# RustAudio/lewton

Hardware: AMD Instinct MI355X
Metric: audio packets/sec (44.1 kHz stereo, 2048-pt long blocks) (higher is better)
Workload: dtype f32; 1 GPU; BASELINE configs[1]: batches of 4096 synthetic 44.1 kHz stereo long-block (n=2048) packets per GPU = 256 streams x 16 consecutive packets, 8 batches rotated, records resident in HBM; streams_per_batch=256, channels=2, blocksize=2048, output=i16 planar, kernels=k_long, parity=unchecked (bench.py --full checks the timed batch against the oracle), parallelism=streams sharded across GPUs, no collectives

## Files before the change

### lewton_amd/csrc/lw_kernels_long.hip

```cpp
#include <algorithm>
#include <cstddef>
#include <mutex>

#include "lw_fast.hpp"
#include "lw_kernels.hpp"
#include "lw_pcm_store.inc"

#define LW_WG (64 * LW_FAST_WAVES)
#define LW_PRIO_FLOOR 2
#define LW_PRIO_IMDCT 0
#define LW_PRIO_FINISH 3
#define LW_FLOOR_FIRST_FROM 7
#define LW_IMDCT_PRIO_LATE 12
#define LW_PRIO_PACE 0
#define LW_PRIO_READY 3
#define LW_SCR_BYTES 4096u
#define LW_PUB_BYTES 4096u
#define LW_LDS_BYTES (LWI_TOTAL + LW_FAST_WAVES * (LW_SCR_BYTES + LW_PUB_BYTES) + 3 * LW_FAST_WAVES * 4)

#include "lw_stamps.inc"

struct LwFastArgs {
	const float *residue;
	const uint16_t *floors;
// ... 11 lines not shown
	float *td;
	float *halo;
	float *edge;
	void *out;
	uint32_t state_stride, state_chan_stride;
	uint32_t edge_n;
	const float *tabA;
	const uint16_t *sid12;
	uint32_t pre[LW_FAST_WAVES];
};
static_assert(offsetof(LwFastArgs, waves) == 48, "kernel reads waves[] through the kernarg segment pointer");

typedef unsigned int uint2_t __attribute__((ext_vector_type(2)));

__device__ __forceinline__ void lds_fence()
{
	asm volatile("" ::: "memory");
}

typedef __attribute__((address_space(3))) const float *lds_cfloat_ptr;
__device__ __forceinline__ float lds_abs_f32(uint32_t byte_addr)
{
	return *reinterpret_cast<lds_cfloat_ptr>((uintptr_t)byte_addr);
}

__device__ __forceinline__ float2_t lds2(const char *base, uint32_t byte_off)
{
	return *reinterpret_cast<const float2_t *>(base + byte_off);
}

__device__ __forceinline__ float4_t lds4(const char *base, uint32_t byte_off)
{
	return *reinterpret_cast<const float4_t *>(base + byte_off);
}

#define LW_PK(name, op, mods)                                                              \
	__device__ __forceinline__ float2_t name(float2_t a, float2_t b)                       \
	{                                                                                      \
		float2_t d;                                                                        \
		asm(op " %0, %1, %2 " mods : "=v"(d) : "v"(a), "v"(b));                            \
		return d;                                                                          \
	}
LW_PK(pk_add, "v_pk_add_f32", "")
LW_PK(pk_sub, "v_pk_add_f32", "neg_lo:[0,1] neg_hi:[0,1]")
LW_PK(pk_add_A2, "v_pk_add_f32", "op_sel:[0,1] op_sel_hi:[1,0] neg_lo:[0,1]")
LW_PK(pk_add_A3, "v_pk_add_f32", "op_sel:[1,1] op_sel_hi:[0,0] neg_lo:[0,1] neg_hi:[1,0]")
LW_PK(pk_add_A4, "v_pk_add_f32", "op_sel:[0,0] op_sel_hi:[1,1] neg_lo:[1,0] neg_hi:[0,1]")
LW_PK(pk_add_A5, "v_pk_add_f32", "op_sel:[1,0] op_sel_hi:[1,0] neg_lo:[0,1]")
LW_PK(pk_add_A6, "v_pk_add_f32", "op_sel:[0,1] op_sel_hi:[1,0] neg_hi:[0,1]")
LW_PK(pk_add_A7, "v_pk_add_f32", "neg_hi:[0,1]")
LW_PK(pk_add_A8, "v_pk_add_f32", "neg_lo:[0,1]")
LW_PK(pk_add_A9, "v_pk_add_f32", "neg_lo:[0,1] neg_hi:[1,0]")
LW_PK(pk_mul, "v_pk_mul_f32", "")
LW_PK(pk_mul_M1, "v_pk_mul_f32", "op_sel:[0,0] op_sel_hi:[1,0]")
LW_PK(pk_mul_M2, "v_pk_mul_f32", "op_sel:[1,1] op_sel_hi:[0,1] neg_hi:[0,1]")
LW_PK(pk_mul_M3, "v_pk_mul_f32", "op_sel:[0,1] op_sel_hi:[0,0]")
LW_PK(pk_mul_M4, "v_pk_mul_f32", "op_sel:[0,0] op_sel_hi:[0,1] neg_hi:[0,1]")
LW_PK(pk_mul_M5, "v_pk_mul_f32", "op_sel:[1,1] op_sel_hi:[1,0] neg_lo:[1,0] neg_hi:[1,0]")
LW_PK(pk_mul_M6, "v_pk_mul_f32", "op_sel:[1,0] op_sel_hi:[1,1] neg_lo:[1,0]")
LW_PK(pk_mul_M7, "v_pk_mul_f32", "op_sel:[0,1] op_sel_hi:[1,1]")
LW_PK(pk_mul_M8, "v_pk_mul_f32", "op_sel:[1,0] op_sel_hi:[0,0] neg_lo:[0,1]")
LW_PK(pk_mul_M9, "v_pk_mul_f32", "op_sel:[1,1] op_sel_hi:[1,0] neg_hi:[1,0]")
LW_PK(pk_mul_M10, "v_pk_mul_f32", "op_sel:[0,0] op_sel_hi:[0,1] neg_lo:[0,1] neg_hi:[0,1]")
LW_PK(pk_mul_M12lo, "v_pk_mul_f32", "op_sel:[0,1] op_sel_hi:[0,0]")
LW_PK(pk_mul_M12hi, "v_pk_mul_f32", "op_sel:[1,1] op_sel_hi:[1,0]")

// ... 195 lines not shown
	    : "+v"(m0), "+v"(a0), "+v"(m1), "+v"(a1), "+v"(m2), "+v"(a2), "+v"(m3), "+v"(a3), "=&v"(t0), "=&v"(t1), "=&v"(t2), "=&v"(t3),
	      "=&s"(c0), "=&s"(c1), "=&s"(c2), "=&s"(c3), "=&s"(d0), "=&s"(d1), "=&s"(d2), "=&s"(d3));
}

struct ItemRegs {
	uint32_t res_off, floor_off, out_off, src_arg;
	int32_t state_out;
	uint32_t halo_out, src_kind, flags;
	uint32_t pkt;
};

struct Pref {
	float4_t r[2][4];
	uint32_t fe[2];
};


__device__ __forceinline__ void issue_floor_loads(const LwFastArgs &F, const ItemRegs &it, const LwFastUnit &un, uint32_t lane,
		Pref &p)
{
	const uint16_t *f0 = F.floors + it.floor_off + (uint32_t)un.ch_a * F.fstride;
	p.fe[0] = lane < un.F_a ? (uint32_t)f0[lane] : 0u;
	p.fe[1] = 0u;
	if (un.ch_b >= 0) {
		const uint16_t *f1 = F.floors + it.floor_off + (uint32_t)un.ch_b * F.fstride;
		p.fe[1] = lane < un.F_b ? (uint32_t)f1[lane] : 0u;
	}
}

template <bool PAIR = false, bool NT = true>
__device__ __forceinline__ void issue_residue_loads(const LwFastArgs &F, const ItemRegs &it, const LwFastUnit &un,
		uint32_t lane, Pref &p)
{
	const float4_t *s0 = reinterpret_cast<const float4_t *>(F.residue + it.res_off + (uint32_t)un.ch_a * 1024u);
#pragma unroll
	for (int x = 0; x < 4; x++)
		p.r[0][x] = NT ? __builtin_nontemporal_load(&s0[64 * x + lane]) : s0[64 * x + lane];
	if (PAIR || un.ch_b >= 0) {
		const float4_t *s1 = reinterpret_cast<const float4_t *>(F.residue + it.res_off + (uint32_t)un.ch_b * 1024u);
#pragma unroll
		for (int x = 0; x < 4; x++)
			p.r[1][x] = NT ? __builtin_nontemporal_load(&s1[64 * x + lane]) : s1[64 * x + lane];
	}
}

template <bool NT = true>
__device__ __forceinline__ void issue_loads(const LwFastArgs &F, const ItemRegs &it, const LwFastUnit &un, uint32_t lane, Pref &p)
{
	issue_residue_loads<false, NT>(F, it, un, lane, p);
	issue_floor_loads(F, it, un, lane, p);
}

struct PreRegs {
	float4_t t[2][4];
};

__device__ __forceinline__ void issue_pre_loads(const LwFastArgs &F, const ItemRegs &it, uint32_t prog, uint32_t lane, PreRegs &q)
{
#pragma unroll
	for (int k = 0; k < 2; k++) {
		const uint32_t c = (prog >> (8 * k)) & 0xffu;
		if (c != LW_PRE_NO_CH) {
			const float4_t *s = reinterpret_cast<const float4_t *>(F.residue + it.res_off + c * 1024u);
#pragma unroll
			for (int x = 0; x < 4; x++)
				q.t[k][x] = s[64 * x + lane];
		} else {
#pragma unroll
			for (int x = 0; x < 4; x++)
				asm volatile("" : "=v"(q.t[k][x]));
		}
	}
}

#define LW_FLOOR_W0 2097153.0f
// ... 79 lines not shown
		ent[(b) & 1][3] = lds4(t, sw.y >> 16);                                         \
	} while (0)
#define LW_SP_XI(b)                                                                    \
	do {                                                                               \
		_Pragma("unroll") for (int j = 0; j < 4; j++) {                                \
			fl[(b) & 1][j] = floor_bin(kf0 + (float)(256 * ((b) & 3) + j), ent[(b) & 1][j]); \
		}                                                                              \
	} while (0)
#define LW_SP_M(b)                                                                     \
	do {                                                                               \
		float4_t &rr = r[(b) >> 2][(b) & 3];                                           \
		const float2_t lo2 = pk_mul(float2_t{fl[(b) & 1][0], fl[(b) & 1][1]}, float2_t{rr.x, rr.y}); \
		const float2_t hi2 = pk_mul(float2_t{fl[(b) & 1][2], fl[(b) & 1][3]}, float2_t{rr.z, rr.w}); \
		rr = float4_t{lo2.x, lo2.y, hi2.x, hi2.y};                                     \
	} while (0)
	LW_SP_G(0);
	LW_SP_G(1);
	__builtin_amdgcn_sched_barrier(0);
#pragma unroll
	for (int b = 0; b < 8; b++) {
		LW_SP_XI(b);
		if (b + 2 < 8)
			LW_SP_G(b + 2);
		if (b >= 1)
			LW_SP_M(b - 1);
		__builtin_amdgcn_sched_barrier(0);
	}
	LW_SP_M(7);
#undef LW_SP_G
#undef LW_SP_XI
#undef LW_SP_M
}

__device__ __forceinline__ void floor_values(const char *img, const char *sc, uint32_t lane, uint32_t fslot, bool unused,
		float4_t (&fl)[4])
{
	if (unused) {
#pragma unroll
		for (int x = 0; x < 4; x++)
			fl[x] = float4_t{0.0f, 0.0f, 0.0f, 0.0f};
		return;
	}
	const float kf0 = (float)(4 * (int)lane);
#pragma unroll
	for (int x = 0; x < 4; x++) {
		const uint2_t sw = *reinterpret_cast<const uint2_t *>(img + LWI_SID16 + 8u * ((fslot * 4 + x) * 64u + lane));
		const uint32_t s16[4] = {sw.x & 0xffffu, sw.x >> 16, sw.y & 0xffffu, sw.y >> 16};
#pragma unroll
		for (int j = 0; j < 4; j++) {
			fl[x][j] = floor_bin(kf0 + (float)(256 * x + j), lds4(sc, s16[j]));
		}
	}
}

template <int NCH>
__device__ __forceinline__ void floor_phase(const LwFastArgs &F, const char *img, char *sc, uint32_t lane, const LwFastUnit &un,
		const uint32_t (&fe)[2], float4_t (&fl)[2][4])
{
	__builtin_amdgcn_s_setprio(LW_PRIO_FLOOR);
	const bool unused0 = floor_table(F, img, sc, lane, fe[0], un.floor_a, un.F_a);
	bool unused1 = false;
	if (NCH == 2)
		unused1 = floor_table(F, img, sc + 1024, lane, fe[1], un.floor_b, un.F_b);
	lds_fence();
	floor_values(img, sc, lane, un.floor_a, unused0, fl[0]);
	if (NCH == 2)
		floor_values(img, sc + 1024, lane, un.floor_b, unused1, fl[1]);
	lds_fence();
	__builtin_amdgcn_s_setprio(0);
}

template <int NCH>
__device__ __forceinline__ void stage_b(const LwFastArgs &F, const char *img, uint32_t lane, const float4_t (&r)[2][4],
		float2_t (&P)[2][8])
{
	const uint32_t mirror = (63u - lane) << 2;
	float2_t au[4], al[4];
#pragma unroll
	for (int x = 0; x < 4; x++) {
		const uint32_t m = 64u * x + lane;
		au[x] = lds2(img + LWI_APAIR, 8u * m);
		al[x] = lds2(img + LWI_APAIR, 8u * (511u - m));
	}
#pragma unroll
	for (int c = 0; c < NCH; c++) {
		float2_t U[4];
		step1x2(r[c][0], au[0], al[0], r[c][1], au[1], al[1], U[0], P[c][0], U[1], P[c][1]);
		step1x2(r[c][2], au[2], al[2], r[c][3], au[3], al[3], U[2], P[c][2], U[3], P[c][3]);
#pragma unroll
		for (int x = 0; x < 4; x++) {
			P[c][7 - x].x = __int_as_float(__builtin_amdgcn_ds_bpermute(mirror, __float_as_int(U[x].x)));
			P[c][7 - x].y = __int_as_float(__builtin_amdgcn_ds_bpermute(mirror, __float_as_int(U[x].y)));
		}
	}
	float2_t s2[4], l0[2], l1;
#pragma unroll
	for (int x = 0; x < 4; x++)
		s2[x] = lds2(img + LWI_TW_S2, 8u * (64u * x + lane));
	l0[0] = lds2(img + LWI_TW_L0, 8u * lane);
	l0[1] = lds2(img + LWI_TW_L0, 8u * (64u + lane));
// ... 239 lines not shown
	float2_t P0[8], P1[8];
	TwC tc;
	{
		TwB tb;
		load_tw_b(img, lane, tb);
		stage_b1(tb, lane, r[0], P0);
		stage_b1(tb, lane, r[1], P1);
		load_tw_c(img, lane, tc);
		t2_inreg(P0);
		t2_inreg(P1);
		__builtin_amdgcn_sched_barrier(0);
	}
	stage_c1(tc, P0);
	__builtin_amdgcn_sched_barrier(0);
	const float a2s = *reinterpret_cast<const float *>(img + LWI_A2);
	const float2_t a2 = float2_t{a2s, a2s};
	t3_inreg(P0);
	stage_c1(tc, P1);
	__builtin_amdgcn_sched_barrier(0);
	t3_inreg(P1);
	stage_d_block(a2, P0);
	__builtin_amdgcn_sched_barrier(0);
	t4_write(sc, lane, P0);
	__builtin_amdgcn_sched_barrier(0);
	stage_e1(img, sc, lane, R[0]);
	stage_d_block(a2, P1);
	__builtin_amdgcn_sched_barrier(0);
	t4_write(sc, lane, P1);
	__builtin_amdgcn_sched_barrier(0);
	stage_e1(img, sc, lane, R[1]);
	__builtin_amdgcn_sched_barrier(0);
}

__device__ __forceinline__ void decouple_pair(Pref &pf)
{
#pragma unroll
	for (int x = 0; x < 4; x++) {
		float m[4] = {pf.r[0][x].x, pf.r[0][x].y, pf.r[0][x].z, pf.r[0][x].w};
		float a[4] = {pf.r[1][x].x, pf.r[1][x].y, pf.r[1][x].z, pf.r[1][x].w};
		decouple4(m[0], a[0], m[1], a[1], m[2], a[2], m[3], a[3]);
		pf.r[0][x] = float4_t{m[0], m[1], m[2], m[3]};
		pf.r[1][x] = float4_t{a[0], a[1], a[2], a[3]};
	}
}

__device__ __forceinline__ void couple_quad(float4_t &M, float4_t &A)
{
	float m[4] = {M.x, M.y, M.z, M.w};
	float a[4] = {A.x, A.y, A.z, A.w};
	decouple4_branchy(m[0], a[0], m[1], a[1], m[2], a[2], m[3], a[3]);
	M = float4_t{m[0], m[1], m[2], m[3]};
	A = float4_t{a[0], a[1], a[2], a[3]};
}

__device__ __forceinline__ void apply_pre(uint32_t prog, Pref &pf, PreRegs &q)
{
	const uint32_t n = prog >> 28;
#pragma unroll
	for (int x = 0; x < 4; x++) {
		float4_t v0 = pf.r[0][x], v1 = pf.r[1][x], v2 = q.t[0][x], v3 = q.t[1][x];
#pragma nounroll
		for (uint32_t i = 0; i < n; i++) {
			switch ((prog >> (16u + 4u * i)) & 0xfu) {
			case 0x1: couple_quad(v0, v1); break;
			case 0x2: couple_quad(v0, v2); break;
			case 0x3: couple_quad(v0, v3); break;
			case 0x4: couple_quad(v1, v0); break;
			case 0x6: couple_quad(v1, v2); break;
			case 0x7: couple_quad(v1, v3); break;
			case 0x8: couple_quad(v2, v0); break;
			case 0x9: couple_quad(v2, v1); break;
			case 0xb: couple_quad(v2, v3); break;
			case 0xc: couple_quad(v3, v0); break;
			case 0xd: couple_quad(v3, v1); break;
			case 0xe: couple_quad(v3, v2); break;
			default: break;
			}
		}
		pf.r[0][x] = v0;
		pf.r[1][x] = v1;
	}
}

template <int NCH, bool SPLIT = false>
__device__ __forceinline__ void spectrum_fused(const LwFastArgs &F, const char *img, char *sc, uint32_t lane,
		const LwFastUnit &un, Pref &pf)
{
	__builtin_amdgcn_s_setprio(LW_PRIO_FLOOR);
	const bool unused0 = floor_table(F, img, sc, lane, pf.fe[0], un.floor_a, un.F_a);
	bool unused1 = false;
	if (NCH == 2)
		unused1 = floor_table(F, img, sc + 1024, lane, pf.fe[1], un.floor_b, un.F_b);
	lds_fence();
	if (NCH == 2 && un.coupled)
		decouple_pair(pf);
	if (SPLIT && NCH == 1 && un.coupled >= LW_UNIT_SPLIT_MAG) {
		if (un.coupled == LW_UNIT_SPLIT_ANG) {
#pragma unroll
			for (int x = 0; x < 4; x++) {
				const float4_t t = pf.r[0][x];
				pf.r[0][x] = pf.r[1][x];
				pf.r[1][x] = t;
			}
			decouple_pair(pf);
#pragma unroll
			for (int x = 0; x < 4; x++)
				pf.r[0][x] = pf.r[1][x];
		} else {
			decouple_pair(pf);
		}
	}
	if (NCH == 2 && !unused0 && !unused1) {
		spectrum_pair(img, sc, lane, un.floor_a, un.floor_b, pf.r);
	} else {
		spectrum(F, img, sc, lane, un.floor_a, unused0, pf.r[0]);
		if (NCH == 2)
			spectrum(F, img, sc + 1024, lane, un.floor_b, unused1, pf.r[1]);
	}
	lds_fence();
}

__device__ __forceinline__ void spectrum_ready(const LwFastUnit &un, Pref &pf, const float4_t (&fl)[2][4])
{
	if (un.coupled)
		decouple_pair(pf);
#pragma unroll
	for (int c = 0; c < 2; c++)
#pragma unroll
		for (int x = 0; x < 4; x++) {
			const float2_t lo2 = pk_mul(float2_t{fl[c][x].x, fl[c][x].y}, float2_t{pf.r[c][x].x, pf.r[c][x].y});
			const float2_t hi2 = pk_mul(float2_t{fl[c][x].z, fl[c][x].w}, float2_t{pf.r[c][x].z, pf.r[c][x].w});
			pf.r[c][x] = float4_t{lo2.x, lo2.y, hi2.x, hi2.y};
		}
}

template <int NCH, int UP = 0>
__device__ __forceinline__ void long_imdct(const LwFastArgs &F, const char *img, char *sc, uint32_t lane, Pref &pf,
		float2_t (&R)[2][2][4])
{
	if (__builtin_amdgcn_readfirstlane(threadIdx.x >> 6) >= LW_IMDCT_PRIO_LATE)
		__builtin_amdgcn_s_setprio(LW_PRIO_IMDCT + 1 + UP);
	else
		__builtin_amdgcn_s_setprio(LW_PRIO_IMDCT + UP);
	if (NCH == 2) {
		imdct_pair(img, sc, lane, pf.r, R);
		return;
	}
	float2_t P[2][8];
	stage_b<NCH>(F, img, lane, pf.r, P);
#pragma unroll
	for (int c = 0; c < NCH; c++)
		t2_inreg(P[c]);
	stage_c<NCH>(F, img, lane, P);
#pragma unroll
	for (int c = 0; c < NCH; c++) {
		t3_inreg(P[c]);
	}
	{
		const float a2s = *reinterpret_cast<const float *>(img + LWI_A2);
		const float2_t a2 = float2_t{a2s, a2s};
#pragma unroll
		for (int c = 0; c < NCH; c++)
			stage_d_block(a2, P[c]);
	}
#pragma unroll
	for (int c = 0; c < NCH; c++) {
		t4_write(sc, lane, P[c]);
		lds_fence();
#pragma unroll
		for (int c2 = 0; c2 < 2; c2++) {
			TwidE te;
			te.Cq = lds4(img + LWI_C4, 16u * (64u * c2 + lane));
			te.Bl = lds4(img + LWI_B_LO, 16u * (64u * c2 + lane));
// ... 6 lines not shown

template <int NCH>
__device__ __forceinline__ void publish(char *dst, uint32_t lane, const float2_t (&R)[2][2][4])
{
#pragma unroll
	for (int c = 0; c < 2; c++)
		if (c < NCH) {
#pragma unroll
			for (int c2 = 0; c2 < 2; c2++)
				*reinterpret_cast<float4_t *>(dst + 2048 * c + 16u * (64u * c2 + lane)) =
					float4_t{R[c][c2][0].y, R[c][c2][1].y, R[c][c2][2].y, R[c][c2][3].y};
		}
}

#define LW_PB_LO0(c) float4_t{R[c][0][3].y, R[c][0][2].y, R[c][1][3].y, R[c][1][2].y}
#define LW_PB_LO1(c) float4_t{R[c][1][1].y, R[c][1][0].y, R[c][0][1].y, R[c][0][0].y}

struct PrevHalf {
	float2_t pp[2][2];
};

__device__ __forceinline__ void prev_from_lds(const char *src, uint32_t lane, PrevHalf &h)
{
#pragma unroll
	for (int c2 = 0; c2 < 2; c2++) {
		const float4_t v = *reinterpret_cast<const float4_t *>(src + 16u * (64u * c2 + lane));
		h.pp[c2][0] = float2_t{v.x, v.y};
		h.pp[c2][1] = float2_t{v.z, v.w};
	}
}

__device__ __forceinline__ void prev_from_global(const float *g, uint32_t lane, PrevHalf &h)
{
	const float4_t g0 = *reinterpret_cast<const float4_t *>(g + 4u * lane);
	const float4_t g1 = *reinterpret_cast<const float4_t *>(g + 508u - 4u * lane);
	h.pp[0][1] = float2_t{g0.y, g0.x};
	h.pp[1][1] = float2_t{g0.w, g0.z};
	h.pp[1][0] = float2_t{g1.y, g1.x};
	h.pp[0][0] = float2_t{g1.w, g1.z};
}

__device__ __forceinline__ void ola_pack_i16(const char *img, uint32_t lane, const float2_t (&Rc)[2][4], const PrevHalf &h,
		uint32_t (&D)[4][2])
{
	float2_t O[2][4];
#pragma unroll
	for (int c2 = 0; c2 < 2; c2++) {
		const float4_t w0 = lds4(img + LWI_WIN, 32u * (64u * c2 + lane));
		const float4_t w1 = lds4(img + LWI_WIN, 32u * (64u * c2 + lane) + 16u);
		ola_block<true>(Rc[c2], h.pp[c2][0], h.pp[c2][1], w0, w1, O[c2]);
	}
	typedef short short2_t __attribute__((ext_vector_type(2)));
	union {
		short2_t s;
		uint32_t u;
	} a;
#define LW_PKI(d, v0, v1) a.s = __builtin_amdgcn_cvt_pk_i16((int)(v0), (int)(v1)), d = a.u
	LW_PKI(D[0][0], O[0][3].x, O[0][2].x);
	LW_PKI(D[0][1], O[1][3].x, O[1][2].x);
	LW_PKI(D[1][0], O[1][1].x, O[1][0].x);
	LW_PKI(D[1][1], O[0][1].x, O[0][0].x);
	LW_PKI(D[2][0], O[0][0].y, O[0][1].y);
	LW_PKI(D[2][1], O[1][0].y, O[1][1].y);
	LW_PKI(D[3][0], O[1][2].y, O[1][3].y);
	LW_PKI(D[3][1], O[0][2].y, O[0][3].y);
#undef LW_PKI
}

__device__ __forceinline__ void store_interleaved2(const LwFastArgs &F, uint32_t lane, uint32_t out_off,
		const uint32_t (&L)[4][2], const uint32_t (&R)[4][2])
{
	int16_t *o = reinterpret_cast<int16_t *>(F.out) + out_off;
	const uint32_t pos[4] = {4u * lane, 508u - 4u * lane, 512u + 4u * lane, 1020u - 4u * lane};
#pragma unroll
	for (int g = 0; g < 4; g++) {
		const uint32_t d0 = __builtin_amdgcn_perm(R[g][0], L[g][0], 0x05040100u);
		const uint32_t d1 = __builtin_amdgcn_perm(R[g][0], L[g][0], 0x07060302u);
		const uint32_t d2 = __builtin_amdgcn_perm(R[g][1], L[g][1], 0x05040100u);
		const uint32_t d3 = __builtin_amdgcn_perm(R[g][1], L[g][1], 0x07060302u);
		store16_wt(o + 2u * pos[g], float4_t{__uint_as_float(d0), __uint_as_float(d1), __uint_as_float(d2), __uint_as_float(d3)});
	}
}

__device__ __forceinline__ void ola_quads_f32(const char *img, uint32_t lane, const float2_t (&Rc)[2][4], const PrevHalf &h, float4_t (&V)[4])
{
	float2_t O[2][4];
#pragma unroll
	for (int c2 = 0; c2 < 2; c2++) {
		const float4_t w0 = lds4(img + LWI_WIN, 32u * (64u * c2 + lane));
		const float4_t w1 = lds4(img + LWI_WIN, 32u * (64u * c2 + lane) + 16u);
		ola_block<false>(Rc[c2], h.pp[c2][0], h.pp[c2][1], w0, w1, O[c2]);
	}
	const LwQuads q = pcm_quads(O);
#pragma unroll
	for (int g = 0; g < 4; g++)
		V[g] = float4_t{q.v[g][0], q.v[g][1], q.v[g][2], q.v[g][3]};
}

__device__ __forceinline__ void store_interleaved2_f32(const LwFastArgs &F, uint32_t lane, uint32_t out_off, const float4_t (&L)[4],
		const float4_t (&R)[4])
{
	float *o = reinterpret_cast<float *>(F.out) + out_off;
	const bool odd = (lane & 1u) != 0;
#pragma unroll
	for (int g = 0; g < 4; g++) {
		const uint32_t b = 256u * (uint32_t)g;
#pragma unroll
		for (int h = 0; h < 2; h++) {
			const uint32_t k = 32u * (uint32_t)h + (lane >> 1);
			const int src = (int)((g & 1) ? 63u - k : k) << 2;
#define LW_BP(v) __int_as_float(__builtin_amdgcn_ds_bpermute(src, __float_as_int(v)))
			const float lx = LW_BP(L[g].x), ly = LW_BP(L[g].y), lz = LW_BP(L[g].z), lw = LW_BP(L[g].w);
			const float rx = LW_BP(R[g].x), ry = LW_BP(R[g].y), rz = LW_BP(R[g].z), rw = LW_BP(R[g].w);
#undef LW_BP
			const float4_t v = odd ? float4_t{lz, rz, lw, rw} : float4_t{lx, rx, ly, ry};
			store16_wt(o + 2u * (b + 128u * (uint32_t)h + 2u * lane), v);
		}
	}
}

template <int FMT>
__device__ __forceinline__ void ola_store(const LwFastArgs &F, const char *img, uint32_t lane, int chn,
		uint32_t out_off, const float2_t (&Rc)[2][4], const PrevHalf &h, uint32_t mch = 1024u)
{
	float2_t O[2][4];
#pragma unroll
	for (int c2 = 0; c2 < 2; c2++) {
		const float4_t w0 = lds4(img + LWI_WIN, 32u * (64u * c2 + lane));
		const float4_t w1 = lds4(img + LWI_WIN, 32u * (64u * c2 + lane) + 16u);
		ola_block<!lw_out_f32(FMT)>(Rc[c2], h.pp[c2][0], h.pp[c2][1], w0, w1, O[c2]);
	}
	const uint32_t p0 = 4u * lane, p1 = 508u - 4u * lane, p2 = 512u + 4u * lane, p3 = 1020u - 4u * lane;
	if (FMT == LW_OUT_F32_PLANAR) {
		float *o = reinterpret_cast<float *>(F.out) + out_off + (uint32_t)chn * mch;
		store16_wt(o + p0, float4_t{O[0][3].x, O[0][2].x, O[1][3].x, O[1][2].x});
		store16_wt(o + p1, float4_t{O[1][1].x, O[1][0].x, O[0][1].x, O[0][0].x});
		store16_wt(o + p2, float4_t{O[0][0].y, O[0][1].y, O[1][0].y, O[1][1].y});
		store16_wt(o + p3, float4_t{O[1][2].y, O[1][3].y, O[0][2].y, O[0][3].y});
	} else if (FMT == LW_OUT_F32_INTERLEAVED) {
		float *o = reinterpret_cast<float *>(F.out) + out_off + (uint32_t)chn;
		const uint32_t pos[4] = {p0, p1, p2, p3};
		const float v[4][4] = {{O[0][3].x, O[0][2].x, O[1][3].x, O[1][2].x}, {O[1][1].x, O[1][0].x, O[0][1].x, O[0][0].x},
			{O[0][0].y, O[0][1].y, O[1][0].y, O[1][1].y}, {O[1][2].y, O[1][3].y, O[0][2].y, O[0][3].y}};
#pragma unroll
		for (int g = 0; g < 4; g++) {
			uint32_t off = pos[g] * F.ch;
			asm volatile("" : "+v"(off));
#pragma unroll
			for (int k = 0; k < 4; k++) {
				o[off] = v[g][k];
				off += F.ch;
			}
		}
	} else {
		int iq[2][4], im[2][4];
#pragma unroll
		for (int c2 = 0; c2 < 2; c2++)
#pragma unroll
			for (int k = 0; k < 4; k++) {
				iq[c2][k] = (int)O[c2][k].x;
				im[c2][k] = (int)O[c2][k].y;
			}
		if (FMT == LW_OUT_I16_PLANAR) {
			typedef short short2_t __attribute__((ext_vector_type(2)));
			union {
				short2_t s;
				uint32_t u;
			} a, b;
			int16_t *o = reinterpret_cast<int16_t *>(F.out) + out_off + (uint32_t)chn * mch;
			{
			a.s = __builtin_amdgcn_cvt_pk_i16(iq[0][3], iq[0][2]);
			b.s = __builtin_amdgcn_cvt_pk_i16(iq[1][3], iq[1][2]);
			store_pcm8(o + p0, a.u, b.u);
			a.s = __builtin_amdgcn_cvt_pk_i16(iq[1][1], iq[1][0]);
			b.s = __builtin_amdgcn_cvt_pk_i16(iq[0][1], iq[0][0]);
			store_pcm8(o + p1, a.u, b.u);
			a.s = __builtin_amdgcn_cvt_pk_i16(im[0][0], im[0][1]);
			b.s = __builtin_amdgcn_cvt_pk_i16(im[1][0], im[1][1]);
			store_pcm8(o + p2, a.u, b.u);
			a.s = __builtin_amdgcn_cvt_pk_i16(im[1][2], im[1][3]);
			b.s = __builtin_amdgcn_cvt_pk_i16(im[0][2], im[0][3]);
			store_pcm8(o + p3, a.u, b.u);
			}
		} else {
			typedef short short2_t __attribute__((ext_vector_type(2)));
			int16_t *o = reinterpret_cast<int16_t *>(F.out) + out_off + (uint32_t)chn;
			const uint32_t pos[4] = {p0, p1, p2, p3};
			const int lo[4][2] = {{iq[0][3], iq[1][3]}, {iq[1][1], iq[0][1]}, {im[0][0], im[1][0]}, {im[1][2], im[0][2]}};
			const int hi[4][2] = {{iq[0][2], iq[1][2]}, {iq[1][0], iq[0][0]}, {im[0][1], im[1][1]}, {im[1][3], im[0][3]}};
#pragma unroll
			for (int g = 0; g < 4; g++) {
				uint32_t off = pos[g] * F.ch;
				asm volatile("" : "+v"(off));
#pragma unroll
				for (int h2 = 0; h2 < 2; h2++) {
					const short2_t pk = __builtin_amdgcn_cvt_pk_i16(lo[g][h2], hi[g][h2]);
					o[off] = pk.x;
					off += F.ch;
					o[off] = pk.y;
					off += F.ch;
				}
			}
		}
	}
}

#define LW_PA_LO0(c) float4_t{R[c][0][3].x, R[c][0][2].x, R[c][1][3].x, R[c][1][2].x}
#define LW_PA_LO1(c) float4_t{R[c][1][1].x, R[c][1][0].x, R[c][0][1].x, R[c][0][0].x}
__device__ __forceinline__ void store_left_half(float *dst, uint32_t lane, float4_t lo0, float4_t lo1)
{
	const float4_t hi0 = float4_t{-lo1.w, -lo1.z, -lo1.y, -lo1.x};
	const float4_t hi1 = float4_t{-lo0.w, -lo0.z, -lo0.y, -lo0.x};
	store16_wt(dst + 4u * lane, lo0);
	store16_wt(dst + 508u - 4u * lane, lo1);
	store16_wt(dst + 512u + 4u * lane, hi0);
	store16_wt(dst + 1020u - 4u * lane, hi1);
}

__device__ __forceinline__ void store_right_half(float *dst, uint32_t lane, float4_t lo0, float4_t lo1)
{
	const float4_t hi0 = float4_t{lo1.w, lo1.z, lo1.y, lo1.x};
	const float4_t hi1 = float4_t{lo0.w, lo0.z, lo0.y, lo0.x};
	store16_wt(dst + 4u * lane, lo0);
	store16_wt(dst + 508u - 4u * lane, lo1);
	store16_wt(dst + 512u + 4u * lane, hi0);
	store16_wt(dst + 1020u - 4u * lane, hi1);
}

template <int FMT>
__device__ __forceinline__ void store_quad(const LwFastArgs &F, int chn, uint32_t out_off, uint32_t mch, uint32_t rel, float4_t v, bool valid)
{
	if (!valid)
		return;
	if (FMT == LW_OUT_F32_PLANAR) {
		store16_wt(reinterpret_cast<float *>(F.out) + out_off + (uint32_t)chn * mch + rel, v);
		return;
	}
	if (FMT == LW_OUT_F32_INTERLEAVED) {
		float *o = reinterpret_cast<float *>(F.out) + out_off + rel * F.ch + (uint32_t)chn;
		o[0] = v.x;
		o[F.ch] = v.y;
		o[2u * F.ch] = v.z;
		o[3u * F.ch] = v.w;
		return;
	}
	typedef short short2_t __attribute__((ext_vector_type(2)));
	const float2_t k = float2_t{32768.0f, 32768.0f};
	const float2_t lo = pk_mul(float2_t{v.x, v.y}, k), hi = pk_mul(float2_t{v.z, v.w}, k);
	union {
		short2_t s;
		uint32_t u;
	} a, b;
	a.s = __builtin_amdgcn_cvt_pk_i16((int)lo.x, (int)lo.y);
	b.s = __builtin_amdgcn_cvt_pk_i16((int)hi.x, (int)hi.y);
	int16_t *o = reinterpret_cast<int16_t *>(F.out) + out_off;
	if (FMT == LW_OUT_I16_PLANAR) {
		store_pcm8(o + (uint32_t)chn * mch + rel, a.u, b.u);
	} else {
		uint32_t off = rel * F.ch + (uint32_t)chn;
// ... 713 lines not shown
```

### lewton_amd/csrc/lw_long_body.inc

```
	extern __shared__ __attribute__((aligned(16))) char smem[];
	const uint32_t lane_id = threadIdx.x & 63u;
	const uint32_t wave = __builtin_amdgcn_readfirstlane(threadIdx.x >> 6);
	LW_STAMP_DECL;
	LW_STAMP(0);
	const uint32_t n_units = F.n_units, per_round = F.per_round, rounds = F.rounds;
	LwFastUnit un;
#if defined(__HIP_DEVICE_COMPILE__)
	typedef const unsigned long long __attribute__((address_space(4))) *ka_ptr;
	const unsigned long long unit_word = ((ka_ptr)__builtin_amdgcn_kernarg_segment_ptr())[offsetof(LwFastArgs, waves) / 8 + wave];
#else
	const unsigned long long unit_word = 0;
#endif
	asm volatile("" ::"s"(F.residue), "s"(F.floors), "s"(F.n_items), "s"(n_units), "s"(per_round), "s"(rounds), "s"(F.dense),
			"s"(F.late_from), "s"(F.ch), "s"(F.fstride), "s"(F.image), "s"(unit_word));
	__builtin_memcpy(&un, &unit_word, 8);
	const uint32_t slot = un.slot, uidx = wave - slot * n_units;
	const bool active = slot < per_round;
	const uint32_t item0 = blockIdx.x * per_round * rounds + slot;
	const bool two = !SPLIT && un.ch_b >= 0;
	const int chn[2] = {un.ch_a, two ? un.ch_b : un.ch_a};
	const uint32_t pre_prog = PRE ? __builtin_amdgcn_readfirstlane(F.pre[wave]) : 0u;
	PreRegs pq;
#define LW_PRE_WAVES 2
	const bool late = !RIGHT_ONLY && wave >= (F.late_from > LW_PRE_WAVES ? F.late_from : (uint32_t)LW_PRE_WAVES);
// ... 31 lines not shown
		dst[LW_WG - 256] = v1;
#ifdef LW_LONG_BODY_STAGE_STORE
		LW_LONG_BODY_STAGE_STORE
#endif
		lds_fence();
		if (valid && !late)
			{
				issue_loads<!PRE>(F, it, un, lane_id, pf);
				if (PRE)
					issue_pre_loads(F, it, pre_prog, lane_id, pq);
			}
		if (valid && floor_first)
			issue_floor_loads(F, it, un, lane_id, pf);
	}
	__syncthreads();
#ifdef LW_LONG_BODY_AFTER_STAGE
	LW_LONG_BODY_AFTER_STAGE
#endif
	const char *img = smem;
	LW_STAMP(2);
	char *sc = smem + LWI_TOTAL + wave * LW_SCR_BYTES;
	char *pub0 = smem + LWI_TOTAL + LW_FAST_WAVES * LW_SCR_BYTES;
	char *pub = pub0 + wave * LW_PUB_BYTES;
#define LW_PACE_VMCNT 63
	const bool paced = !RIGHT_ONLY && F.late_from < LW_FAST_WAVES;
	uint32_t lane0 = lane_id;
	asm volatile("" : "+v"(lane0));
	if (valid && floor_first) {
		float4_t fl[2][4];
		floor_phase<2>(F, img, sc, lane0, un, pf.fe, fl);
		LW_STAMP(1);
		__builtin_amdgcn_s_setprio(LW_PRIO_PACE);
		lds_wait_ge(LW_CNT_LANDED(wave - F.late_from), 1u);
		issue_residue_loads<true, !PRE>(F, it, un, lane_id, pf);
		if (PRE)
			issue_pre_loads(F, it, pre_prog, lane_id, pq);
		LW_STAMP(15);
		if (wave + F.late_from < LW_FAST_WAVES) {
			asm volatile("s_waitcnt vmcnt(%0)" ::"n"(LW_PACE_VMCNT) : "memory");
			lds_store_u32(LW_CNT_LANDED(wave), 1u);
		}
		if (F.dense)
			it = load_item(F.items, item0);
		__builtin_amdgcn_s_setprio(LW_PRIO_READY);
		LW_STAMP_W(3);
		if (PRE)
			apply_pre(pre_prog, pf, pq);
		spectrum_ready(un, pf, fl);
		__builtin_amdgcn_s_setprio(0);
		LW_STAMP(4);
	} else {
		if (paced) {
			__builtin_amdgcn_s_setprio(LW_PRIO_PACE);
			if (late) {
				lds_wait_ge(LW_CNT_LANDED(wave - F.late_from), 1u);
				if (valid)
					{
				issue_loads<!PRE>(F, it, un, lane_id, pf);
				if (PRE)
					issue_pre_loads(F, it, pre_prog, lane_id, pq);
			}
			}
			LW_STAMP(15);
			if (wave + F.late_from < LW_FAST_WAVES) {
				asm volatile("s_waitcnt vmcnt(%0)" ::"n"(LW_PACE_VMCNT) : "memory");
				lds_store_u32(LW_CNT_LANDED(wave), 1u);
			}
			__builtin_amdgcn_s_setprio(0);
		}
		if (valid && F.dense)
			it = load_item(F.items, item0);
		LW_STAMP_W(3);
		if (valid) {
			if (PRE)
				apply_pre(pre_prog, pf, pq);
			if (two)
				spectrum_fused<2>(F, img, sc, lane0, un, pf);
			else
				spectrum_fused<1, SPLIT>(F, img, sc, lane0, un, pf);
		}
		LW_STAMP(4);
	}
	uint32_t n_pub_used = 0;
	uint32_t n_got = 0;
	const uint32_t wprev = slot != 0 ? wave - n_units : (per_round - 1) * n_units + uidx;

	for (uint32_t j = 0; j < rounds; j++) {
		uint32_t lane = lane_id;
		asm volatile("" : "+v"(lane));
		float2_t R[2][2][4];
		const uint32_t item_n = item0 + (j + 1) * per_round;
		const bool valid_n = active && j + 1 < rounds && item_n < F.n_items;
		ItemRegs itn{};
		if (valid_n && !F.dense)
			itn = load_item(F.items, item_n);
		if (valid) {
			if (two)
				long_imdct<2, MIXF ? 1 : 0>(F, img, sc, lane, pf, R);
			else
				long_imdct<1, MIXF ? 1 : 0>(F, img, sc, lane, pf, R);
			if (j == 0)
				LW_STAMP(8);
		}
		if (valid) {
			if (RIGHT_ONLY) {
#pragma unroll
				for (int c = 0; c < 2; c++)
					if (c == 0 || two) {
						float *dst = F.halo + ((size_t)it.halo_out * F.ch + chn[c]) * 512u;
						*reinterpret_cast<float4_t *>(dst + 4u * lane) = LW_PB_LO0(c);
						*reinterpret_cast<float4_t *>(dst + 508u - 4u * lane) = LW_PB_LO1(c);
					}
			} else {
				__builtin_amdgcn_s_setprio(LW_PRIO_FINISH);
				const bool edge_l = EDGE && (it.flags & LW_IF_EDGE_L), edge_r = EDGE && (it.flags & LW_IF_EDGE_R);
				const uint32_t e_ls = edge_l ? 448u : 0u, e_m = EDGE ? (edge_r ? 1472u : 1024u) - e_ls : 1024u;
				if (MIXF && (edge_l || edge_r)) {
#pragma unroll
					for (int c = 0; c < 2; c++)
						if ((c == 0 || two) && lane < 16u) {
							float *edge = F.edge + ((size_t)it.pkt * 2u * F.ch + (uint32_t)chn[c]) * LW_EDGE_VALUES;
							if (edge_l)
								store16_wt(edge + 60u - 4u * lane, LW_PA_LO1(c));
							if (edge_r)
								store16_wt(edge + (size_t)F.ch * LW_EDGE_VALUES + 60u - 4u * lane, LW_PB_LO1(c));
						}
					asm volatile("s_waitcnt vmcnt(0)" ::: "memory");
					if (lane == 0 && !mix_drop_flags) {
#pragma unroll
						for (int c = 0; c < 2; c++)
							if (c == 0 || two) {
								uint32_t *fl = edge_flags + ((size_t)it.pkt * 2u) * F.ch + (uint32_t)chn[c];
								if (edge_l)
									__hip_atomic_store(fl, 1u, __ATOMIC_RELAXED, __HIP_MEMORY_SCOPE_AGENT);
								if (edge_r)
									__hip_atomic_store(fl + F.ch, 1u, __ATOMIC_RELAXED, __HIP_MEMORY_SCOPE_AGENT);
							}
					}
				}
				if (it.flags & LW_IF_NEXT_LDS) {
					lds_wait_ge(LW_CNT_ACK(wave), n_pub_used);
					if (two)
						publish<2>(pub, lane, R);
					else
// ... 151 lines not shown
```

Before: 270.0 million packets/s.

## Use scalar-base global stores, shared floor lookup, and asm stereo decoupling

Global stores now use a wave-uniform SGPR base with per-lane byte offsets and immediate offsets, which cuts per-lane 64-bit address arithmetic. When both channels share a floor, the floor curve lookup is done once for both channels. Stereo decoupling is rewritten as hand-written compare/cndmask asm, and the wave index is passed in instead of being recomputed. The risks are extra s_nop padding, asm scheduling barriers, and the correctness of the hand-written inline asm.

```diff
diff --git a/lewton_amd/csrc/lw_kernels_long.hip b/lewton_amd/csrc/lw_kernels_long.hip
--- a/lewton_amd/csrc/lw_kernels_long.hip
+++ b/lewton_amd/csrc/lw_kernels_long.hip
@@ -67,6 +67,29 @@
 __device__ __forceinline__ float4_t lds4(const char *base, uint32_t byte_off)
 {
 	return *reinterpret_cast<const float4_t *>(base + byte_off);
+}
+
+__device__ __forceinline__ unsigned long long uniform_base(const void *base)
+{
+	const uintptr_t b = (uintptr_t)base;
+	const uint2_t w = uint2_t{(uint32_t)__builtin_amdgcn_readfirstlane((uint32_t)b), (uint32_t)__builtin_amdgcn_readfirstlane((uint32_t)(b >> 32))};
+	unsigned long long sb = __builtin_bit_cast(unsigned long long, w);
+	asm volatile("s_nop 4" : "+s"(sb));
+	return sb;
+}
+
+template <int IMM = 0>
+__device__ __forceinline__ void store16_wt_u(unsigned long long sbase, uint32_t byte_off, float4_t v)
+{
+	static_assert(IMM >= 0 && IMM < 4096, "immediate offset of a global instruction");
+	asm volatile("global_store_dwordx4 %0, %1, %2 offset:%3 sc1\n\ts_nop 1" ::"v"(byte_off), "v"(v), "s"(sbase), "n"(IMM) : "memory");
+}
+
+template <int IMM = 0>
+__device__ __forceinline__ void store_pcm8_u(void *base, uint32_t &byte_off, uint32_t lo, uint32_t hi)
+{
+	asm volatile("" : "+v"(byte_off));
+	store_pcm8(reinterpret_cast<char *>(base) + IMM + byte_off, lo, hi);
 }
 
 #define LW_PK(name, op, mods)                                                              \
@@ -328,15 +351,20 @@
 __device__ __forceinline__ void issue_residue_loads(const LwFastArgs &F, const ItemRegs &it, const LwFastUnit &un,
 		uint32_t lane, Pref &p)
 {
+	const uint32_t lo = 16u * lane;
 	const float4_t *s0 = reinterpret_cast<const float4_t *>(F.residue + it.res_off + (uint32_t)un.ch_a * 1024u);
 #pragma unroll
-	for (int x = 0; x < 4; x++)
-		p.r[0][x] = NT ? __builtin_nontemporal_load(&s0[64 * x + lane]) : s0[64 * x + lane];
+	for (int x = 0; x < 4; x++) {
+		const float4_t *q = reinterpret_cast<const float4_t *>(reinterpret_cast<const char *>(s0 + 64 * x) + lo);
+		p.r[0][x] = NT ? __builtin_nontemporal_load(q) : *q;
+	}
 	if (PAIR || un.ch_b >= 0) {
 		const float4_t *s1 = reinterpret_cast<const float4_t *>(F.residue + it.res_off + (uint32_t)un.ch_b * 1024u);
 #pragma unroll
-		for (int x = 0; x < 4; x++)
-			p.r[1][x] = NT ? __builtin_nontemporal_load(&s1[64 * x + lane]) : s1[64 * x + lane];
+		for (int x = 0; x < 4; x++) {
+			const float4_t *q = reinterpret_cast<const float4_t *>(reinterpret_cast<const char *>(s1 + 64 * x) + lo);
+			p.r[1][x] = NT ? __builtin_nontemporal_load(q) : *q;
+		}
 	}
 }
 
@@ -482,6 +510,63 @@
 #undef LW_SP_M
 }
 
+__device__ __forceinline__ void spectrum_pair_shared(const char *img, const char *sc, uint32_t lane, uint32_t fslot, float4_t (&r)[2][4])
+{
+	const float kf0 = (float)(4 * (int)lane);
+	uint2_t sid[4];
+#pragma unroll
+	for (int x = 0; x < 4; x++)
+		sid[x] = *reinterpret_cast<const uint2_t *>(img + LWI_SID16 + 8u * ((fslot * 4 + x) * 64u + lane));
+	const char *ta[4];
+	float kf[4];
+	float4_t ent[2][4];
+	float fl[2][4];
+#define LW_SS_G(b)                                                                     \
+	do {                                                                               \
+		if (((b) & 1) == 0) {                                                          \
+			const uint2_t sw = sid[(b) >> 1];                                          \
+			ta[0] = sc + (sw.x & 0xffffu);                                             \
+			ta[1] = sc + (sw.x >> 16);                                                 \
+			ta[2] = sc + (sw.y & 0xffffu);                                             \
+			ta[3] = sc + (sw.y >> 16);                                                 \
+		}                                                                              \
+		_Pragma("unroll") for (int j = 0; j < 4; j++)                                  \
+			ent[(b) & 1][j] = lds4(ta[j], 1024u * ((b) & 1));                          \
+	} while (0)
+#define LW_SS_XI(b)                                                                    \
+	do {                                                                               \
+		if (((b) & 1) == 0) {                                                          \
+			_Pragma("unroll") for (int j = 0; j < 4; j++)                              \
+				kf[j] = kf0 + (float)(256 * ((b) >> 1) + j);                           \
+		}                                                                              \
+		_Pragma("unroll") for (int j = 0; j < 4; j++)                                  \
+			fl[(b) & 1][j] = floor_bin(kf[j], ent[(b) & 1][j]);                        \
+	} while (0)
+#define LW_SS_M(b)                                                                     \
+	do {                                                                               \
+		float4_t &rr = r[(b) & 1][(b) >> 1];                                           \
+		const float2_t lo2 = pk_mul(float2_t{fl[(b) & 1][0], fl[(b) & 1][1]}, float2_t{rr.x, rr.y}); \
+		const float2_t hi2 = pk_mul(float2_t{fl[(b) & 1][2], fl[(b) & 1][3]}, float2_t{rr.z, rr.w}); \
+		rr = float4_t{lo2.x, lo2.y, hi2.x, hi2.y};                                     \
+	} while (0)
+	LW_SS_G(0);
+	LW_SS_G(1);
+	__builtin_amdgcn_sched_barrier(0);
+#pragma unroll
+	for (int b = 0; b < 8; b++) {
+		LW_SS_XI(b);
+		if (b + 2 < 8)
+			LW_SS_G(b + 2);
+		if (b >= 1)
+			LW_SS_M(b - 1);
+		__builtin_amdgcn_sched_barrier(0);
+	}
+	LW_SS_M(7);
+#undef LW_SS_G
+#undef LW_SS_XI
+#undef LW_SS_M
+}
+
 __device__ __forceinline__ void floor_values(const char *img, const char *sc, uint32_t lane, uint32_t fslot, bool unused,
 		float4_t (&fl)[4])
 {
@@ -499,6 +584,23 @@
 #pragma unroll
 		for (int j = 0; j < 4; j++) {
 			fl[x][j] = floor_bin(kf0 + (float)(256 * x + j), lds4(sc, s16[j]));
+		}
+	}
+}
+
+__device__ __forceinline__ void floor_values_shared(const char *img, const char *sc, uint32_t lane, uint32_t fslot, float4_t (&fl)[2][4])
+{
+	const float kf0 = (float)(4 * (int)lane);
+#pragma unroll
+	for (int x = 0; x < 4; x++) {
+		const uint2_t sw = *reinterpret_cast<const uint2_t *>(img + LWI_SID16 + 8u * ((fslot * 4 + x) * 64u + lane));
+		const uint32_t s16[4] = {sw.x & 0xffffu, sw.x >> 16, sw.y & 0xffffu, sw.y >> 16};
+#pragma unroll
+		for (int j = 0; j < 4; j++) {
+			const char *t = sc + s16[j];
+			const float kf = kf0 + (float)(256 * x + j);
+			fl[0][x][j] = floor_bin(kf, lds4(t, 0u));
+			fl[1][x][j] = floor_bin(kf, lds4(t, 1024u));
 		}
 	}
 }
@@ -513,9 +615,13 @@
 	if (NCH == 2)
 		unused1 = floor_table(F, img, sc + 1024, lane, fe[1], un.floor_b, un.F_b);
 	lds_fence();
-	floor_values(img, sc, lane, un.floor_a, unused0, fl[0]);
-	if (NCH == 2)
-		floor_values(img, sc + 1024, lane, un.floor_b, unused1, fl[1]);
+	if (NCH == 2 && !unused0 && !unused1 && un.floor_a == un.floor_b) {
+		floor_values_shared(img, sc, lane, un.floor_a, fl);
+	} else {
+		floor_values(img, sc, lane, un.floor_a, unused0, fl[0]);
+		if (NCH == 2)
+			floor_values(img, sc + 1024, lane, un.floor_b, unused1, fl[1]);
+	}
 	lds_fence();
 	__builtin_amdgcn_s_setprio(0);
 }
@@ -821,16 +927,32 @@
 	__builtin_amdgcn_sched_barrier(0);
 }
 
+__device__ __forceinline__ void decouple_quads(float4_t &M, float4_t &A)
+{
+	float nm0, na0, nm1, na1, nm2, na2, nm3, na3, t0, t1, t2, t3;
+	unsigned long long c0, c1, c2, c3, d0, d1, d2, d3;
+	asm("v_cmp_lt_f32_e64 %12, 0, %20\n\tv_cmp_lt_f32_e64 %13, 0, %22\n\tv_cmp_lt_f32_e64 %14, 0, %24\n\tv_cmp_lt_f32_e64 %15, 0, %26\n\t"
+	    "v_cmp_lt_f32_e64 %16, 0, %21\n\tv_cmp_lt_f32_e64 %17, 0, %23\n\tv_cmp_lt_f32_e64 %18, 0, %25\n\tv_cmp_lt_f32_e64 %19, 0, %27\n\t"
+	    "s_xnor_b64 %12, %12, %16\n\ts_xnor_b64 %13, %13, %17\n\ts_xnor_b64 %14, %14, %18\n\ts_xnor_b64 %15, %15, %19\n\t"
+	    "v_cndmask_b32_e64 %8, %21, -%21, %12\n\tv_cndmask_b32_e64 %9, %23, -%23, %13\n\t"
+	    "v_cndmask_b32_e64 %10, %25, -%25, %14\n\tv_cndmask_b32_e64 %11, %27, -%27, %15\n\t"
+	    "v_add_f32_e32 %8, %20, %8\n\tv_add_f32_e32 %9, %22, %9\n\tv_add_f32_e32 %10, %24, %10\n\tv_add_f32_e32 %11, %26, %11\n\t"
+	    "v_cndmask_b32_e64 %1, %20, %8, %16\n\tv_cndmask_b32_e64 %3, %22, %9, %17\n\t"
+	    "v_cndmask_b32_e64 %5, %24, %10, %18\n\tv_cndmask_b32_e64 %7, %26, %11, %19\n\t"
+	    "v_cndmask_b32_e64 %0, %8, %20, %16\n\tv_cndmask_b32_e64 %2, %9, %22, %17\n\t"
+	    "v_cndmask_b32_e64 %4, %10, %24, %18\n\tv_cndmask_b32_e64 %6, %11, %26, %19"
+	    : "=&v"(nm0), "=&v"(na0), "=&v"(nm1), "=&v"(na1), "=&v"(nm2), "=&v"(na2), "=&v"(nm3), "=&v"(na3), "=&v"(t0), "=&v"(t1),
+	      "=&v"(t2), "=&v"(t3), "=&s"(c0), "=&s"(c1), "=&s"(c2), "=&s"(c3), "=&s"(d0), "=&s"(d1), "=&s"(d2), "=&s"(d3)
+	    : "v"(M.x), "v"(A.x), "v"(M.y), "v"(A.y), "v"(M.z), "v"(A.z), "v"(M.w), "v"(A.w));
+	M = float4_t{nm0, nm1, nm2, nm3};
+	A = float4_t{na0, na1, na2, na3};
+}
+
 __device__ __forceinline__ void decouple_pair(Pref &pf)
 {
 #pragma unroll
-	for (int x = 0; x < 4; x++) {
-		float m[4] = {pf.r[0][x].x, pf.r[0][x].y, pf.r[0][x].z, pf.r[0][x].w};
-		float a[4] = {pf.r[1][x].x, pf.r[1][x].y, pf.r[1][x].z, pf.r[1][x].w};
-		decouple4(m[0], a[0], m[1], a[1], m[2], a[2], m[3], a[3]);
-		pf.r[0][x] = float4_t{m[0], m[1], m[2], m[3]};
-		pf.r[1][x] = float4_t{a[0], a[1], a[2], a[3]};
-	}
+	for (int x = 0; x < 4; x++)
+		decouple_quads(pf.r[0][x], pf.r[1][x]);
 }
 
 __device__ __forceinline__ void couple_quad(float4_t &M, float4_t &A)
@@ -871,7 +993,7 @@
 	}
 }
 
-template <int NCH, bool SPLIT = false>
+template <int NCH, bool SPLIT = false, bool SHARE = false>
 __device__ __forceinline__ void spectrum_fused(const LwFastArgs &F, const char *img, char *sc, uint32_t lane,
 		const LwFastUnit &un, Pref &pf)
 {
@@ -900,7 +1022,10 @@
 		}
 	}
 	if (NCH == 2 && !unused0 && !unused1) {
-		spectrum_pair(img, sc, lane, un.floor_a, un.floor_b, pf.r);
+		if (SHARE && un.floor_a == un.floor_b)
+			spectrum_pair_shared(img, sc, lane, un.floor_a, pf.r);
+		else
+			spectrum_pair(img, sc, lane, un.floor_a, un.floor_b, pf.r);
 	} else {
 		spectrum(F, img, sc, lane, un.floor_a, unused0, pf.r[0]);
 		if (NCH == 2)
@@ -924,10 +1049,10 @@
 }
 
 template <int NCH, int UP = 0>
-__device__ __forceinline__ void long_imdct(const LwFastArgs &F, const char *img, char *sc, uint32_t lane, Pref &pf,
+__device__ __forceinline__ void long_imdct(const LwFastArgs &F, const char *img, char *sc, uint32_t lane, uint32_t wave, Pref &pf,
 		float2_t (&R)[2][2][4])
 {
-	if (__builtin_amdgcn_readfirstlane(threadIdx.x >> 6) >= LW_IMDCT_PRIO_LATE)
+	if (wave >= LW_IMDCT_PRIO_LATE)
 		__builtin_amdgcn_s_setprio(LW_PRIO_IMDCT + 1 + UP);
 	else
 		__builtin_amdgcn_s_setprio(LW_PRIO_IMDCT + UP);
@@ -1000,8 +1125,11 @@
 
 __device__ __forceinline__ void prev_from_global(const float *g, uint32_t lane, PrevHalf &h)
 {
-	const float4_t g0 = *reinterpret_cast<const float4_t *>(g + 4u * lane);
-	const float4_t g1 = *reinterpret_cast<const float4_t *>(g + 508u - 4u * lane);
+	const char *gb = reinterpret_cast<const char *>(g);
+	uint32_t o0 = 16u * lane, o1 = 2032u - 16u * lane;
+	asm volatile("" : "+v"(o0), "+v"(o1));
+	const float4_t g0 = *reinterpret_cast<const float4_t *>(gb + o0);
+	const float4_t g1 = *reinterpret_cast<const float4_t *>(gb + o1);
 	h.pp[0][1] = float2_t{g0.y, g0.x};
 	h.pp[1][1] = float2_t{g0.w, g0.z};
 	h.pp[1][0] = float2_t{g1.y, g1.x};
@@ -1038,7 +1166,7 @@
 __device__ __forceinline__ void store_interleaved2(const LwFastArgs &F, uint32_t lane, uint32_t out_off,
 		const uint32_t (&L)[4][2], const uint32_t (&R)[4][2])
 {
-	int16_t *o = reinterpret_cast<int16_t *>(F.out) + out_off;
+	const unsigned long long sb = uniform_base(reinterpret_cast<int16_t *>(F.out) + out_off);
 	const uint32_t pos[4] = {4u * lane, 508u - 4u * lane, 512u + 4u * lane, 1020u - 4u * lane};
 #pragma unroll
 	for (int g = 0; g < 4; g++) {
@@ -1046,7 +1174,7 @@
 		const uint32_t d1 = __builtin_amdgcn_perm(R[g][0], L[g][0], 0x07060302u);
 		const uint32_t d2 = __builtin_amdgcn_perm(R[g][1], L[g][1], 0x05040100u);
 		const uint32_t d3 = __builtin_amdgcn_perm(R[g][1], L[g][1], 0x07060302u);
-		store16_wt(o + 2u * pos[g], float4_t{__uint_as_float(d0), __uint_as_float(d1), __uint_as_float(d2), __uint_as_float(d3)});
+		store16_wt_u(sb, 4u * pos[g], float4_t{__uint_as_float(d0), __uint_as_float(d1), __uint_as_float(d2), __uint_as_float(d3)});
 	}
 }
 
@@ -1082,7 +1210,7 @@
 			const float rx = LW_BP(R[g].x), ry = LW_BP(R[g].y), rz = LW_BP(R[g].z), rw = LW_BP(R[g].w);
 #undef LW_BP
 			const float4_t v = odd ? float4_t{lz, rz, lw, rw} : float4_t{lx, rx, ly, ry};
-			store16_wt(o + 2u * (b + 128u * (uint32_t)h + 2u * lane), v);
+			store16_wt_u(uniform_base(o + 2u * (b + 128u * (uint32_t)h)), 16u * lane, v);
 		}
 	}
 }
@@ -1101,10 +1229,11 @@
 	const uint32_t p0 = 4u * lane, p1 = 508u - 4u * lane, p2 = 512u + 4u * lane, p3 = 1020u - 4u * lane;
 	if (FMT == LW_OUT_F32_PLANAR) {
 		float *o = reinterpret_cast<float *>(F.out) + out_off + (uint32_t)chn * mch;
-		store16_wt(o + p0, float4_t{O[0][3].x, O[0][2].x, O[1][3].x, O[1][2].x});
-		store16_wt(o + p1, float4_t{O[1][1].x, O[1][0].x, O[0][1].x, O[0][0].x});
-		store16_wt(o + p2, float4_t{O[0][0].y, O[0][1].y, O[1][0].y, O[1][1].y});
-		store16_wt(o + p3, float4_t{O[1][2].y, O[1][3].y, O[0][2].y, O[0][3].y});
+		const unsigned long long sb = uniform_base(o);
+		store16_wt_u(sb, 4u * p0, float4_t{O[0][3].x, O[0][2].x, O[1][3].x, O[1][2].x});
+		store16_wt_u(sb, 4u * p1, float4_t{O[1][1].x, O[1][0].x, O[0][1].x, O[0][0].x});
+		store16_wt_u<2048>(sb, 4u * p0, float4_t{O[0][0].y, O[0][1].y, O[1][0].y, O[1][1].y});
+		store16_wt_u<2048>(sb, 4u * p1, float4_t{O[1][2].y, O[1][3].y, O[0][2].y, O[0][3].y});
 	} else if (FMT == LW_OUT_F32_INTERLEAVED) {
 		float *o = reinterpret_cast<float *>(F.out) + out_off + (uint32_t)chn;
 		const uint32_t pos[4] = {p0, p1, p2, p3};
@@ -1136,19 +1265,20 @@
 				uint32_t u;
 			} a, b;
 			int16_t *o = reinterpret_cast<int16_t *>(F.out) + out_off + (uint32_t)chn * mch;
+			uint32_t b0 = 2u * p0, b1 = 2u * p1;
 			{
 			a.s = __builtin_amdgcn_cvt_pk_i16(iq[0][3], iq[0][2]);
 			b.s = __builtin_amdgcn_cvt_pk_i16(iq[1][3], iq[1][2]);
-			store_pcm8(o + p0, a.u, b.u);
+			store_pcm8_u(o, b0, a.u, b.u);
 			a.s = __builtin_amdgcn_cvt_pk_i16(iq[1][1], iq[1][0]);
 			b.s = __builtin_amdgcn_cvt_pk_i16(iq[0][1], iq[0][0]);
-			store_pcm8(o + p1, a.u, b.u);
+			store_pcm8_u(o, b1, a.u, b.u);
 			a.s = __builtin_amdgcn_cvt_pk_i16(im[0][0], im[0][1]);
 			b.s = __builtin_amdgcn_cvt_pk_i16(im[1][0], im[1][1]);
-			store_pcm8(o + p2, a.u, b.u);
+			store_pcm8_u<1024>(o, b0, a.u, b.u);
 			a.s = __builtin_amdgcn_cvt_pk_i16(im[1][2], im[1][3]);
 			b.s = __builtin_amdgcn_cvt_pk_i16(im[0][2], im[0][3]);
-			store_pcm8(o + p3, a.u, b.u);
+			store_pcm8_u<1024>(o, b1, a.u, b.u);
 			}
 		} else {
 			typedef short short2_t __attribute__((ext_vector_type(2)));
@@ -1179,20 +1309,22 @@
 {
 	const float4_t hi0 = float4_t{-lo1.w, -lo1.z, -lo1.y, -lo1.x};
 	const float4_t hi1 = float4_t{-lo0.w, -lo0.z, -lo0.y, -lo0.x};
-	store16_wt(dst + 4u * lane, lo0);
-	store16_wt(dst + 508u - 4u * lane, lo1);
-	store16_wt(dst + 512u + 4u * lane, hi0);
-	store16_wt(dst + 1020u - 4u * lane, hi1);
+	const unsigned long long sb = uniform_base(dst);
+	store16_wt_u(sb, 16u * lane, lo0);
+	store16_wt_u(sb, 2032u - 16u * lane, lo1);
+	store16_wt_u<2048>(sb, 16u * lane, hi0);
+	store16_wt_u<2048>(sb, 2032u - 16u * lane, hi1);
 }
 
 __device__ __forceinline__ void store_right_half(float *dst, uint32_t lane, float4_t lo0, float4_t lo1)
 {
 	const float4_t hi0 = float4_t{lo1.w, lo1.z, lo1.y, lo1.x};
 	const float4_t hi1 = float4_t{lo0.w, lo0.z, lo0.y, lo0.x};
-	store16_wt(dst + 4u * lane, lo0);
-	store16_wt(dst + 508u - 4u * lane, lo1);
-	store16_wt(dst + 512u + 4u * lane, hi0);
-	store16_wt(dst + 1020u - 4u * lane, hi1);
+	const unsigned long long sb = uniform_base(dst);
+	store16_wt_u(sb, 16u * lane, lo0);
+	store16_wt_u(sb, 2032u - 16u * lane, lo1);
+	store16_wt_u<2048>(sb, 16u * lane, hi0);
+	store16_wt_u<2048>(sb, 2032u - 16u * lane, hi1);
 }
 
 template <int FMT>
diff --git a/lewton_amd/csrc/lw_long_body.inc b/lewton_amd/csrc/lw_long_body.inc
--- a/lewton_amd/csrc/lw_long_body.inc
+++ b/lewton_amd/csrc/lw_long_body.inc
@@ -87,9 +87,9 @@
 		LW_STAMP(1);
 		__builtin_amdgcn_s_setprio(LW_PRIO_PACE);
 		lds_wait_ge(LW_CNT_LANDED(wave - F.late_from), 1u);
-		issue_residue_loads<true, !PRE>(F, it, un, lane_id, pf);
+		issue_residue_loads<true, !PRE>(F, it, un, lane0, pf);
 		if (PRE)
-			issue_pre_loads(F, it, pre_prog, lane_id, pq);
+			issue_pre_loads(F, it, pre_prog, lane0, pq);
 		LW_STAMP(15);
 		if (wave + F.late_from < LW_FAST_WAVES) {
 			asm volatile("s_waitcnt vmcnt(%0)" ::"n"(LW_PACE_VMCNT) : "memory");
@@ -111,9 +111,9 @@
 				lds_wait_ge(LW_CNT_LANDED(wave - F.late_from), 1u);
 				if (valid)
 					{
-				issue_loads<!PRE>(F, it, un, lane_id, pf);
-				if (PRE)
-					issue_pre_loads(F, it, pre_prog, lane_id, pq);
+				issue_loads<!PRE>(F, it, un, lane0, pf);
+				if (PRE)
+					issue_pre_loads(F, it, pre_prog, lane0, pq);
 			}
 			}
 			LW_STAMP(15);
@@ -130,7 +130,7 @@
 			if (PRE)
 				apply_pre(pre_prog, pf, pq);
 			if (two)
-				spectrum_fused<2>(F, img, sc, lane0, un, pf);
+				spectrum_fused<2, false, true>(F, img, sc, lane0, un, pf);
 			else
 				spectrum_fused<1, SPLIT>(F, img, sc, lane0, un, pf);
 		}
@@ -141,8 +141,8 @@
 	const uint32_t wprev = slot != 0 ? wave - n_units : (per_round - 1) * n_units + uidx;
 
 	for (uint32_t j = 0; j < rounds; j++) {
-		uint32_t lane = lane_id;
-		asm volatile("" : "+v"(lane));
+		asm volatile("" : "+v"(lane0));
+		const uint32_t lane = lane0;
 		float2_t R[2][2][4];
 		const uint32_t item_n = item0 + (j + 1) * per_round;
 		const bool valid_n = active && j + 1 < rounds && item_n < F.n_items;
@@ -151,9 +151,9 @@
 			itn = load_item(F.items, item_n);
 		if (valid) {
 			if (two)
-				long_imdct<2, MIXF ? 1 : 0>(F, img, sc, lane, pf, R);
+				long_imdct<2, MIXF ? 1 : 0>(F, img, sc, lane, wave, pf, R);
 			else
-				long_imdct<1, MIXF ? 1 : 0>(F, img, sc, lane, pf, R);
+				long_imdct<1, MIXF ? 1 : 0>(F, img, sc, lane, wave, pf, R);
 			if (j == 0)
 				LW_STAMP(8);
 		}
@@ -163,8 +163,9 @@
 				for (int c = 0; c < 2; c++)
 					if (c == 0 || two) {
 						float *dst = F.halo + ((size_t)it.halo_out * F.ch + chn[c]) * 512u;
-						*reinterpret_cast<float4_t *>(dst + 4u * lane) = LW_PB_LO0(c);
-						*reinterpret_cast<float4_t *>(dst + 508u - 4u * lane) = LW_PB_LO1(c);
+						char *dstb = reinterpret_cast<char *>(dst);
+						*reinterpret_cast<float4_t *>(dstb + 16u * lane) = LW_PB_LO0(c);
+						*reinterpret_cast<float4_t *>(dstb + (2032u - 16u * lane)) = LW_PB_LO1(c);
 					}
 			} else {
 				__builtin_amdgcn_s_setprio(LW_PRIO_FINISH);
```

Result: faster. 273.6 million packets/s, median of 6 (+1.3%).
